# martius-lab/iCEM

Measured on AMD Instinct MI355X. Metric: traj-steps/sec (N x h), iCEM inner planning loop, higher is better.
Workload: dtype f32 storage; model step 2xfp16 planes (3 products), f32 accumulate

## Files before the change

### icem_amd/build.py

```python
import hashlib
import json
import os
import subprocess
import sys
from concurrent.futures import ThreadPoolExecutor

HERE = os.path.dirname(os.path.abspath(__file__))
CSRC = os.path.join(HERE, "csrc")
UNITS = ["generic_kernels.hip", "plan.hip", "abi.hip", "exchange.hip", "k_sample.hip", "k_rollout.hip", "k_merge.hip",
         "k_iter_small.hip", "icem_rssm.hip", "icem_rssm_split.hip", "k_rollout_wide.hip", "collective.hip", "k_rollout_ahead.hip",
         "k_rollout_wide_split.hip", "k_rollout_hn.hip"]
OUT = os.path.join(HERE, "libicem_hip.so")
OUT_FAULTS = os.path.join(HERE, "libicem_hip_faults.so")
FAULT_UNIT = "exchange.hip"
MARK = b"ICEM_BUILD_HASH="
OBJ = os.path.join(CSRC, "_obj")
FLAGS = ["--offload-arch=gfx950", "-O3", "-std=c++17", "-fPIC", "-Wno-unused-function"]
UNIT_FLAGS = {}
if os.environ.get("ICEM_DEV_SHAPES"):
    FLAGS.append(f"-DICEM_FAST_SHAPES(X)=X({os.environ['ICEM_DEV_SHAPES']})")


def _hipcc() -> str:
    return os.environ.get("HIPCC", "/opt/rocm/bin/hipcc")


def _units():
    return [u for u in UNITS if os.path.exists(os.path.join(CSRC, u))]


def _headers():
    hs = sorted(os.path.join(CSRC, f) for f in os.listdir(CSRC) if f.endswith(".h"))
    return hs + [os.path.join(os.path.dirname(HERE), "include", "icem_hip.h")]


def _digest(paths, extra=""):
    m = hashlib.sha256(extra.encode())
    for p in paths:
        m.update(os.path.basename(p).encode())
        with open(p, "rb") as f:
            m.update(f.read())
    return m.hexdigest()[:16]


def source_hash() -> str:
    return _digest([os.path.join(CSRC, u) for u in _units()] + _headers(), " ".join(FLAGS) + repr(sorted(UNIT_FLAGS.items())))


def embedded_hash(path: str = OUT):
    try:
        with open(path, "rb") as f:
            blob = f.read()
    except OSError:
        return None
    at = blob.find(MARK)
    if at < 0:
        return None
    tag = blob[at + len(MARK):at + len(MARK) + 16]
    return tag.decode() if len(tag) == 16 and all(c in b"0123456789abcdef" for c in tag) else None


def build_info() -> dict:
    info = {"source_hash": source_hash(), "built_from": embedded_hash(), "stale": True}
    info["stale"] = info["built_from"] != info["source_hash"]
    return info


def up_to_date() -> bool:
    return not build_info()["stale"]


def _compile(unit, headers_digest, verbose, faults=False):
    src = os.path.join(CSRC, unit)
    extra = [f'-DICEM_BUILD_HASH="{source_hash()}"'] if unit == "abi.hip" else []
    if faults:
        extra.append("-DICEM_FAULT_INJECTION")
    cmd = [_hipcc(), *FLAGS, *UNIT_FLAGS.get(unit, []), *extra, "-I", CSRC, "-c", src]
    key = _digest([src], " ".join(cmd[1:-1]) + headers_digest)
    stem = os.path.splitext(unit)[0] + ("_faults" if faults else "")
    obj = os.path.join(OBJ, f"{stem}.{key}.o")
    if not os.path.exists(obj):
        for f in os.listdir(OBJ):
            if f.startswith(stem + ".") and f.endswith(".o"):
                os.remove(os.path.join(OBJ, f))
        if verbose:
            print(" ".join(cmd + ["-o", obj]), flush=True)
        subprocess.check_call(cmd + ["-o", obj + ".tmp"])
        os.replace(obj + ".tmp", obj)
    return obj


def build(force: bool = False, verbose: bool = True) -> str:
    if not force and up_to_date() and embedded_hash(OUT_FAULTS) == source_hash():
        return OUT
    os.makedirs(OBJ, exist_ok=True)
    if force:
        for f in os.listdir(OBJ):
            os.remove(os.path.join(OBJ, f))
    hd = _digest(_headers())
    with ThreadPoolExecutor(max_workers=min(8, os.cpu_count() or 1)) as ex:
        fut_faults = ex.submit(_compile, FAULT_UNIT, hd, verbose, True)
        objs = list(ex.map(lambda u: _compile(u, hd, verbose), _units()))
        obj_faults = fut_faults.result()
    objs_f = [obj_faults if os.path.basename(o).startswith(os.path.splitext(FAULT_UNIT)[0] + ".") else o for o in objs]
    for out, oo in ((OUT, objs), (OUT_FAULTS, objs_f)):
        cmd = [_hipcc(), "--offload-arch=gfx950", "-shared", "-fPIC", *oo, "-ldl", "-o", out]
        if verbose:
            print(" ".join(cmd), flush=True)
        subprocess.check_call(cmd)
    if embedded_hash() != source_hash():
        raise RuntimeError("libicem_hip.so does not carry the hash of the sources it was just built from")
    return OUT


if __name__ == "__main__":
    build(force="--force" in sys.argv)
    print(json.dumps(build_info()))
```

### icem_amd/csrc/fused_dev.h

```cpp
#pragma once
#include "icem_fused.h"

#include <climits>
#include <cmath>
#include <cstdlib>
#include <algorithm>
#include <type_traits>
#include <utility>

#include "exchange_dev.h"
#include "philox.h"
#include "refit.h"

#ifndef ICEM_FAST_SHAPES
#define ICEM_FAST_SHAPES(X) X(30, 6, 17) X(30, 6, 18) X(12, 6, 17) X(13, 4, 17) X(30, 17, 24)
#endif
#define ICEM_FAST_HORIZONS(X) X(30) X(12) X(13) X(10)

namespace icem {

namespace {

constexpr int HMAX = 32;
constexpr int SWG = 256;
// ... 1036 lines not shown

__device__ __forceinline__ unsigned long long wave_min_u64(unsigned long long x) {
    x = min_dpp<0xB1, 0xF>(x);
    x = min_dpp<0x4E, 0xF>(x);
    x = min_dpp<0x141, 0xF>(x);
    x = min_dpp<0x140, 0xF>(x);
    x = min_dpp<0x142, 0xA>(x);
    x = min_dpp<0x143, 0xC>(x);
    const unsigned lo = __builtin_amdgcn_readlane((int)(unsigned)x, 63);
    const unsigned hi = __builtin_amdgcn_readlane((int)(unsigned)(x >> 32), 63);
    return ((unsigned long long)hi << 32) | lo;
}

template <int CTRL, int ROW_MASK>
__device__ __forceinline__ unsigned min_dpp32(unsigned x) {
    const unsigned o = (unsigned)__builtin_amdgcn_update_dpp((int)x, (int)x, CTRL, ROW_MASK, 0xF, false);
    return o < x ? o : x;
}
__device__ __forceinline__ unsigned wave_min_u32(unsigned x) {
    x = min_dpp32<0xB1, 0xF>(x);
    x = min_dpp32<0x4E, 0xF>(x);
    x = min_dpp32<0x141, 0xF>(x);
    x = min_dpp32<0x140, 0xF>(x);
    x = min_dpp32<0x142, 0xA>(x);
    x = min_dpp32<0x143, 0xC>(x);
    return (unsigned)__builtin_amdgcn_readlane((int)x, 63);
}
__device__ __forceinline__ unsigned long long wave_min_key(unsigned long long x) {
    const unsigned hi = (unsigned)(x >> 32), lo = (unsigned)x;
    const unsigned mh = wave_min_u32(hi);
    const unsigned long long tie = __ballot(hi == mh);
    unsigned ml;
    if (__popcll(tie) == 1)
        ml = (unsigned)__builtin_amdgcn_readlane((int)lo, __ffsll((long long)tie) - 1);
    else
        ml = wave_min_u32(hi == mh ? lo : 0xFFFFFFFFu);
    return ((unsigned long long)mh << 32) | ml;
}

template <int CTRL, int ROW_MASK>
__device__ __forceinline__ unsigned add_dpp(unsigned x) {
    return x + (unsigned)__builtin_amdgcn_update_dpp(0, (int)x, CTRL, ROW_MASK, 0xF, ROW_MASK == 0xF);
}
__device__ __forceinline__ unsigned wave_incl_scan_u32(unsigned x) {
    x = add_dpp<0x111, 0xF>(x);
    x = add_dpp<0x112, 0xF>(x);
    x = add_dpp<0x114, 0xF>(x);
    x = add_dpp<0x118, 0xF>(x);
    x = add_dpp<0x142, 0xA>(x);
    x = add_dpp<0x143, 0xC>(x);
    return x;
}

__device__ __forceinline__ int keep_index0(const MergeSingleArgs& a) { return a.keep_base >= 0 ? a.keep_base : a.n_global; }

template <int KREG>
__device__ __forceinline__ void merge_select(const MergeSingleArgs& a, int lane, unsigned long long* cand,
                                             unsigned long long* sel) {
    unsigned long long k[LPL][KREG];
    const float keep_cost = a.elites_cost_cur ? a.elites_cost_cur[lane < a.n_keep ? lane : 0] : 0.f;
#pragma unroll
    for (int l = 0; l < LPL; ++l) {
        const int list = lane + l * 64;
#pragma unroll
        for (int i = 0; i < KREG; ++i)
            k[l][i] = a.part_k[(size_t)(i < a.K ? i : 0) * a.n_lists + (list < a.n_lists ? list : 0)];
    }
#pragma unroll
    for (int l = 0; l < LPL; ++l) {
        const bool has_list = lane + l * 64 < a.n_lists;
#pragma unroll
        for (int i = 0; i < KREG; ++i) k[l][i] = (has_list && i < a.K) ? k[l][i] : KEY_SENTINEL;
    }
    if (a.dbg && threadIdx.x == 0) a.dbg[1] = wall_clock64();
    if (lane < a.n_keep) {
        unsigned long long v = make_key(keep_cost, keep_index0(a) + lane);
#pragma unroll
        for (int i = 0; i < KREG; ++i) {
            const bool sw = v < k[0][i];
            const unsigned long long t = sw ? k[0][i] : v;
            k[0][i] = sw ? v : k[0][i];
            v = t;
        }
    }
    if (a.dbg && threadIdx.x == 0) a.dbg[2] = wall_clock64();
    unsigned long long mine = k[0][0];
#pragma unroll
    for (int l = 1; l < LPL; ++l) mine = k[l][0] < mine ? k[l][0] : mine;
    const unsigned srt = wave_sort64_u32((unsigned)(mine >> 32), lane);
    const unsigned T = __shfl(srt, a.K - 1, 64);
    unsigned n_cand = 0;
#pragma unroll
    for (int i = 0; i < KREG; ++i) {
        bool p[LPL];
        bool any_lane = false;
#pragma unroll
        for (int l = 0; l < LPL; ++l) {
            p[l] = (unsigned)(k[l][i] >> 32) <= T && k[l][i] != KEY_SENTINEL;
            any_lane |= p[l];
        }
        if (__ballot(any_lane) == 0) break;
#pragma unroll
        for (int l = 0; l < LPL; ++l) {
            const unsigned long long m = __ballot(p[l]);
            if (m != 0) {
                const unsigned pos = n_cand + __builtin_amdgcn_mbcnt_hi((unsigned)(m >> 32), __builtin_amdgcn_mbcnt_lo((unsigned)m, 0u));
                if (p[l] && pos < 64) cand[pos] = k[l][i];
                n_cand += (unsigned)__popcll(m);
            }
        }
    }
    if (a.dbg && threadIdx.x == 0) a.dbg[3] = wall_clock64();
    __builtin_amdgcn_fence(__ATOMIC_SEQ_CST, "workgroup");
    if (n_cand <= 64) {
        unsigned long long key = lane < (int)n_cand ? *((volatile unsigned long long*)&cand[lane]) : KEY_SENTINEL;
        key = wave_sort_n(key, lane, n_cand);
        if (lane < a.K) sel[lane] = key;
    } else {
        for (int r = 0; r < a.K; ++r) {
            unsigned long long head = k[0][0];
#pragma unroll
            for (int l = 1; l < LPL; ++l) head = k[l][0] < head ? k[l][0] : head;
            const unsigned long long best = wave_min_u64(head);
            if (best != KEY_SENTINEL) {
#pragma unroll
                for (int l = 0; l < LPL; ++l) {
                    if (k[l][0] == best) {
#pragma unroll
                        for (int i = 0; i + 1 < KREG; ++i) k[l][i] = k[l][i + 1];
                        k[l][KREG - 1] = KEY_SENTINEL;
                    }
                }
            }
            if (lane == 0) sel[r] = best;
        }
    }
}

__device__ __forceinline__ void merge_select_stream(const MergeSingleArgs& a, int lane, unsigned long long* cand,
                                                    unsigned long long* sel) {
    const int K = a.K, nl = a.n_lists;
    auto key_at = [&](int l, int i) -> unsigned long long {
        const int list = lane + l * 64;
        const unsigned long long v = a.part_k[(size_t)(i < K ? i : 0) * nl + (list < nl ? list : 0)];
        return (list < nl && i < K) ? v : KEY_SENTINEL;
    };
    const unsigned long long kept = lane < a.n_keep ? make_key(a.elites_cost_cur[lane], keep_index0(a) + lane) : KEY_SENTINEL;
    unsigned long long mine = kept;
#pragma unroll
    for (int l = 0; l < LPL; ++l) {
        const unsigned long long v = key_at(l, 0);
        mine = v < mine ? v : mine;
    }
    const unsigned long long srt = wave_sort64(mine, lane);
    const unsigned long long T = __shfl(srt, K - 1, 64);
    unsigned n_cand = 0;
    auto offer = [&](unsigned long long key) {
        const bool p = key <= T && key != KEY_SENTINEL;
        const unsigned long long m = __ballot(p);
        if (m != 0) {
            const unsigned pos = n_cand + __builtin_amdgcn_mbcnt_hi((unsigned)(m >> 32), __builtin_amdgcn_mbcnt_lo((unsigned)m, 0u));
            if (p && pos < 64) cand[pos] = key;
            n_cand += (unsigned)__popcll(m);
        }
        return m != 0;
    };
    offer(kept);
#pragma unroll 1
    for (int l = 0; l < LPL; ++l) {
        if (l * 64 >= nl) break;
#pragma unroll 1
        for (int i = 0; i < K; ++i)
            if (!offer(key_at(l, i))) break;
    }
    __builtin_amdgcn_fence(__ATOMIC_SEQ_CST, "workgroup");
    if (n_cand <= 64) {
        unsigned long long key = lane < (int)n_cand ? *((volatile unsigned long long*)&cand[lane]) : KEY_SENTINEL;
        key = wave_sort_n(key, lane, n_cand);
        if (lane < K) sel[lane] = key;
    } else {
        int cur[LPL];
#pragma unroll
        for (int l = 0; l < LPL; ++l) cur[l] = 0;
        bool kept_live = true;
        for (int r = 0; r < K; ++r) {
            unsigned long long head = kept_live ? kept : KEY_SENTINEL;
#pragma unroll
            for (int l = 0; l < LPL; ++l) {
                const unsigned long long v = key_at(l, cur[l]);
                head = v < head ? v : head;
            }
            const unsigned long long best = wave_min_u64(head);
            if (best != KEY_SENTINEL) {
                if (kept_live && kept == best) kept_live = false;
#pragma unroll
                for (int l = 0; l < LPL; ++l)
                    if (key_at(l, cur[l]) == best) ++cur[l];
            }
            if (lane == 0) sel[r] = best;
        }
    }
}

template <int DEPTH>
__device__ __forceinline__ void merge_select_shallow(const MergeSingleArgs& a, int lane, unsigned long long* cand,
                                                     unsigned long long* sel) {
    const int K = a.K, nl = a.n_lists;
    const float keep_cost = a.elites_cost_cur ? a.elites_cost_cur[lane < a.n_keep ? lane : 0] : 0.f;
    unsigned long long k[LPL][DEPTH];
#pragma unroll
    for (int l = 0; l < LPL; ++l) {
        const int list = lane + l * 64;
#pragma unroll
        for (int i = 0; i < DEPTH; ++i) k[l][i] = a.part_k[(size_t)(i < K ? i : 0) * nl + (list < nl ? list : 0)];
    }
#pragma unroll
    for (int l = 0; l < LPL; ++l) {
        const bool has_list = lane + l * 64 < nl;
#pragma unroll
        for (int i = 0; i < DEPTH; ++i) k[l][i] = (has_list && i < K) ? k[l][i] : KEY_SENTINEL;
    }
    const unsigned long long kept = lane < a.n_keep ? make_key(keep_cost, keep_index0(a) + lane) : KEY_SENTINEL;
    unsigned long long mine = k[0][0];
#pragma unroll
    for (int l = 1; l < LPL; ++l) mine = k[l][0] < mine ? k[l][0] : mine;
    const unsigned srt = wave_sort64_u32((unsigned)(mine >> 32), lane);
    const unsigned T = __shfl(srt, K - 1, 64);
    unsigned n_cand = 0;
    auto offer = [&](unsigned long long key) {
        const bool p = (unsigned)(key >> 32) <= T && key != KEY_SENTINEL;
        const unsigned long long m = __ballot(p);
        if (m != 0) {
            const unsigned pos = n_cand + __builtin_amdgcn_mbcnt_hi((unsigned)(m >> 32), __builtin_amdgcn_mbcnt_lo((unsigned)m, 0u));
            if (p && pos < 64) cand[pos] = key;
            n_cand += (unsigned)__popcll(m);
        }
        return m != 0;
    };
    bool deeper[LPL];
#pragma unroll
    for (int l = 0; l < LPL; ++l) {
        deeper[l] = true;
#pragma unroll
        for (int i = 0; i < DEPTH; ++i)
            if (deeper[l]) deeper[l] = offer(k[l][i]);
    }
#pragma unroll 1
    for (int l = 0; l < LPL; ++l) {
        if (!deeper[l]) continue;
#pragma unroll 1
        for (int i = DEPTH; i < K; ++i) {
            const int list = lane + l * 64;
            const unsigned long long v = list < nl ? a.part_k[(size_t)i * nl + list] : KEY_SENTINEL;
            if (!offer(v)) break;
        }
    }
    offer(kept);
    __builtin_amdgcn_fence(__ATOMIC_SEQ_CST, "workgroup");
    if (n_cand <= 64) {
        unsigned long long key = lane < (int)n_cand ? *((volatile unsigned long long*)&cand[lane]) : KEY_SENTINEL;
        key = wave_sort_n(key, lane, n_cand);
        if (lane < K) sel[lane] = key;
    } else {
        merge_select_stream(a, lane, cand, sel);
    }
}

__device__ __forceinline__ void merge_select_records(const MergeSingleArgs& a, int lane, unsigned long long* cand,
                                                     unsigned long long* sel, int* slot, long long* stamp = nullptr) {
    const int K = a.K, rs = a.h * a.d + 2;
    xchg_wait(a.xw, lane);
    if (stamp && lane == 0) *stamp = wall_clock64();
    auto rec_key = [&](int e) -> unsigned long long {
        if (e >= a.n_rec) return KEY_SENTINEL;
        const float* rec = a.records + (size_t)e * rs;
        return make_key(rec[0], reinterpret_cast<const int*>(rec + 1)[0]);
    };
    unsigned long long k[3] = {rec_key(lane), rec_key(lane + 64),
                               lane < a.n_keep ? make_key(a.elites_cost_cur[lane], a.n_global + lane) : KEY_SENTINEL};
    const unsigned long long k0 = k[0], k1 = k[1], k2 = k[2];
    for (int r = 0; r < K; ++r) {
        unsigned long long head = k[0] < k[1] ? k[0] : k[1];
        head = k[2] < head ? k[2] : head;
        const unsigned long long best = wave_min_key(head);
        if (best != KEY_SENTINEL) {
            if (k0 == best) { slot[r] = lane; k[0] = KEY_SENTINEL; }
            if (k1 == best) { slot[r] = lane + 64; k[1] = KEY_SENTINEL; }
            if (k2 == best) { slot[r] = a.n_rec + lane; k[2] = KEY_SENTINEL; }
        } else if (lane == 0) {
            slot[r] = 0;
        }
        if (lane == 0) sel[r] = best;
    }
    (void)cand;
}

__device__ __forceinline__ void merge_select_records_wg(const MergeSingleArgs& a, bool stager, int lane, int tid, int nthr,
                                                        unsigned long long* sel, int* slot, long long* stamp = nullptr) {
    __shared__ unsigned long long rk_keys[192];
    __shared__ unsigned rk_rank[192];
    const int K = a.K, rs = a.h * a.d + 2;
    if (stager) {
        xchg_wait(a.xw, lane);
        if (stamp && lane == 0) *stamp = wall_clock64();
        auto rec_key = [&](int e) -> unsigned long long {
            if (e >= a.n_rec) return KEY_SENTINEL;
            const float* rec = a.records + (size_t)e * rs;
            return make_key(rec[0], reinterpret_cast<const int*>(rec + 1)[0]);
        };
        rk_keys[lane] = rec_key(lane);
        rk_keys[64 + lane] = rec_key(lane + 64);
        rk_keys[128 + lane] = lane < a.n_keep ? make_key(a.elites_cost_cur[lane], a.n_global + lane) : KEY_SENTINEL;
        rk_rank[lane] = rk_rank[64 + lane] = rk_rank[128 + lane] = 0u;
// ... 9 lines not shown
        const int c = tid % n_live, p = tid / n_live;
        const unsigned long long mine = rk_keys[at(c)];
        unsigned cnt = 0;
        for (int j = p; j < n_live; j += parts) cnt += rk_keys[at(j)] < mine ? 1u : 0u;
        if (cnt) atomicAdd(&rk_rank[at(c)], cnt);
    }
    if (n_live > nthr)
        for (int c = nthr + tid; c < n_live; c += nthr) {
            const unsigned long long mine = rk_keys[at(c)];
            unsigned cnt = 0;
            for (int j = 0; j < n_live; ++j) cnt += rk_keys[at(j)] < mine ? 1u : 0u;
            rk_rank[at(c)] = cnt;
        }
    __syncthreads();
    for (int c = tid; c < n_live; c += nthr) {
        const unsigned long long mine = rk_keys[at(c)];
        const unsigned r = rk_rank[at(c)];
        if (mine != KEY_SENTINEL && r < (unsigned)K) {
            sel[r] = mine;
            slot[r] = c;
        }
    }
    __syncthreads();
}

template <int KREG>
__device__ __forceinline__ void merge_select_split_stage1(const MergeSingleArgs& a, int lane, int w, int nw, unsigned long long* cand ,
                                                          unsigned long long* wsel ) {
    const int per = (a.n_lists + nw - 1) / nw;
    const int base = w * per;
    const int cnt = base < a.n_lists ? (a.n_lists - base < per ? a.n_lists - base : per) : 0;
    const bool has = lane < cnt;
    const int list = has ? base + lane : 0;
    unsigned long long k[KREG];
#pragma unroll
    for (int i = 0; i < KREG; ++i) k[i] = a.part_k[(size_t)(i < a.K ? i : 0) * a.n_lists + list];
#pragma unroll
    for (int i = 0; i < KREG; ++i) k[i] = (has && i < a.K) ? k[i] : KEY_SENTINEL;
    const unsigned srt = wave_sort64_u32((unsigned)(k[0] >> 32), lane);
    const unsigned T = __shfl(srt, a.K - 1, 64);
    unsigned n_cand = 0;
#pragma unroll
    for (int i = 0; i < KREG; ++i) {
        const bool p = (unsigned)(k[i] >> 32) <= T && k[i] != KEY_SENTINEL;
        const unsigned long long m = __ballot(p);
        if (m == 0) break;
        const unsigned pos = n_cand + __builtin_amdgcn_mbcnt_hi((unsigned)(m >> 32), __builtin_amdgcn_mbcnt_lo((unsigned)m, 0u));
        if (p && pos < 64) cand[pos] = k[i];
        n_cand += (unsigned)__popcll(m);
    }
    __builtin_amdgcn_fence(__ATOMIC_SEQ_CST, "workgroup");
    unsigned long long* out = wsel + w * 16;
    if (n_cand <= 64) {
        unsigned long long key = lane < (int)n_cand ? *((volatile unsigned long long*)&cand[lane]) : KEY_SENTINEL;
        key = wave_sort_n(key, lane, n_cand);
        if (lane < 16) out[lane] = lane < a.K ? key : KEY_SENTINEL;
    } else {
        for (int r = 0; r < a.K; ++r) {
            const unsigned long long best = wave_min_u64(k[0]);
            if (best != KEY_SENTINEL && k[0] == best) {
#pragma unroll
                for (int i = 0; i + 1 < KREG; ++i) k[i] = k[i + 1];
                k[KREG - 1] = KEY_SENTINEL;
            }
            if (lane == 0) out[r] = best;
        }
        if (lane >= a.K && lane < 16) out[lane] = KEY_SENTINEL;
    }
}
__device__ __forceinline__ float merge_keep_cost(const MergeSingleArgs& a, int lane) {
    return a.elites_cost_cur ? a.elites_cost_cur[lane < a.n_keep ? lane : 0] : 0.f;
}
__device__ __forceinline__ void merge_select_split_stage2(const MergeSingleArgs& a, int lane, int nw, const unsigned long long* wsel,
                                                          unsigned long long* cand, unsigned long long* sel, float keep_cost) {
    unsigned long long k[5];
#pragma unroll
    for (int j = 0; j < 4; ++j) k[j] = (lane + 64 * j < nw * 16) ? *((volatile const unsigned long long*)&wsel[lane + 64 * j]) : KEY_SENTINEL;
    k[4] = (lane < a.n_keep && a.elites_cost_cur) ? make_key(keep_cost, keep_index0(a) + lane) : KEY_SENTINEL;
    unsigned long long mine = k[0];
#pragma unroll
    for (int j = 1; j < 5; ++j) mine = k[j] < mine ? k[j] : mine;
    const unsigned long long srt = wave_sort64(mine, lane);
    const unsigned long long T = __shfl(srt, a.K - 1, 64);
    unsigned n_cand = 0;
#pragma unroll
    for (int j = 0; j < 5; ++j) {
        const bool p = k[j] <= T && k[j] != KEY_SENTINEL;
        const unsigned long long m = __ballot(p);
        const unsigned pos = n_cand + __builtin_amdgcn_mbcnt_hi((unsigned)(m >> 32), __builtin_amdgcn_mbcnt_lo((unsigned)m, 0u));
        if (p && pos < 64) cand[pos] = k[j];
        n_cand += (unsigned)__popcll(m);
    }
    __builtin_amdgcn_fence(__ATOMIC_SEQ_CST, "workgroup");
    if (n_cand <= 64) {
        unsigned long long key = lane < (int)n_cand ? *((volatile unsigned long long*)&cand[lane]) : KEY_SENTINEL;
        key = wave_sort_n(key, lane, n_cand);
        if (lane < a.K) sel[lane] = key;
    } else {
        for (int r = 0; r < a.K; ++r) {
            unsigned long long head = k[0];
#pragma unroll
            for (int j = 1; j < 5; ++j) head = k[j] < head ? k[j] : head;
            const unsigned long long best = wave_min_u64(head);
            if (best != KEY_SENTINEL) {
#pragma unroll
                for (int j = 0; j < 5; ++j)
                    if (k[j] == best) k[j] = KEY_SENTINEL;
            }
            if (lane == 0) sel[r] = best;
        }
    }
}

template <int NW>
__device__ __forceinline__ bool merge_select_split_by_rank(const MergeSingleArgs& a) { return a.n_keep <= (16 - a.K) * NW; }
template <int NW>
__device__ __forceinline__ float merge_keep_cost_split(const MergeSingleArgs& a, int lane, int w) {
    const int j = w + NW * (lane - a.K);
    return a.elites_cost_cur ? a.elites_cost_cur[(lane >= a.K && lane < 16 && j < a.n_keep) ? j : 0] : 0.f;
}
template <int NW>
__device__ __forceinline__ void merge_select_split_keep(const MergeSingleArgs& a, int lane, int w, unsigned long long* wsel,
                                                        unsigned long long* sel, float keep_cost) {
    if (lane >= a.K && lane < 16) {
        const int j = w + NW * (lane - a.K);
        wsel[w * 16 + lane] = (j < a.n_keep && a.elites_cost_cur) ? make_key(keep_cost, keep_index0(a) + j) : KEY_SENTINEL;
    }
    if (w == 0 && lane < 16) sel[lane] = KEY_SENTINEL;
}
template <int NW>
__device__ __forceinline__ void merge_select_split_rank(const MergeSingleArgs& a, int lane, int w, const unsigned long long* wsel,
                                                        unsigned long long* sel) {
    typedef unsigned long long u64x2 __attribute__((ext_vector_type(2)));
    const int i = lane & 15, q = lane >> 4;
    const unsigned long long mine = wsel[w * 16 + i];
    const u64x2* pairs = reinterpret_cast<const u64x2*>(wsel) + q;
    unsigned place = 0;
#pragma unroll
    for (int c = 0; c < 2 * NW; ++c) {
        const u64x2 b = pairs[4 * c];
        place += (b[0] < mine ? 1u : 0u) + (b[1] < mine ? 1u : 0u);
    }
    place += (unsigned)__shfl_xor((int)place, 16, 64);
    place += (unsigned)__shfl_xor((int)place, 32, 64);
    if (q == 0 && mine != KEY_SENTINEL && place < (unsigned)a.K) sel[place] = mine;
}

template <int KREG, bool REC>
__device__ __forceinline__ void merge_rows(const MergeSingleArgs& a, const unsigned long long* sel, const int* slot,
                                           const float* (&rows)[KREG]) {
    const int hd = a.h * a.d;
    const int lane = (int)(threadIdx.x & 63);
    const int v = REC ? slot[lane < a.K ? lane : 0] : key_idx(sel[lane < a.K ? lane : 0]);
    const float* mine;
    if (REC) mine = v < a.n_rec ? a.records + (size_t)v * (hd + 2) + 2 : a.elites_cur + (size_t)(v - a.n_rec) * hd;
    else mine = v < a.n_pool ? a.actions + (size_t)v * hd : a.elites_cur + (size_t)(v - a.n_global) * hd;
    const unsigned long long bits = (unsigned long long)(size_t)mine;
#pragma unroll
    for (int r = 0; r < KREG; ++r) {
        const int rr = r < a.K ? r : 0;
        const unsigned lo = (unsigned)__builtin_amdgcn_readlane((int)(unsigned)bits, rr);
        const unsigned hi = (unsigned)__builtin_amdgcn_readlane((int)(unsigned)(bits >> 32), rr);
        rows[r] = reinterpret_cast<const float*>((size_t)(((unsigned long long)hi << 32) | lo));
    }
}

template <int H, int D, int ROUNDS, bool RAW>
__device__ __forceinline__ void sample_into_tile(const FastSampleArgs& sa, int n_rows, int r_mine, int jd, float* trow,
                                                 const float* mrow) {
    constexpr int HD = H * D;
    if (r_mine < sa.n) {
        if (RAW) {
            sample_row<H, ROUNDS>(sa.W, (unsigned)(sa.first_index + r_mine), (unsigned)jd, sa.off_lo, sa.off_hi,
                                  sa.seed_lo, sa.seed_hi, [&](int t, float y) { trow[t * D] = y; }, sa.white != 0);
        } else {
            const float lo = sa.low[jd], hi = sa.high[jd];
            sample_row<H, ROUNDS>(sa.W, (unsigned)(sa.first_index + r_mine), (unsigned)jd, sa.off_lo, sa.off_hi,
                                  sa.seed_lo, sa.seed_hi, [&](int t, float y) {
                                      const float v = __builtin_fmaf(y, mrow[HD + t * D], mrow[t * D]);
                                      trow[t * D] = __builtin_amdgcn_fmed3f(v, lo, hi);
                                  }, sa.white != 0);
        }
    } else if (r_mine < n_rows && !RAW) {
        const int e = r_mine - sa.n;
        const float lo = sa.low[jd], hi = sa.high[jd];
        float last = 0.f;
        sample_row<H, ROUNDS>(sa.W, (unsigned)e, (unsigned)jd, sa.off2_lo, sa.off2_hi, sa.seed_lo, sa.seed_hi,
                              [&](int t, float y) {
                                  if (t == H - 1) {
                                      const float v = __builtin_fmaf(y, mrow[HD + t * D], mrow[t * D]);
                                      last = __builtin_amdgcn_fmed3f(v, lo, hi);
                                  }
                              }, sa.white != 0);
        const float* src = sa.elites_src + (size_t)e * HD + jd;
        for (int t = 0; t < H - 1; ++t) trow[t * D] = src[(t + 1) * D];
        trow[(H - 1) * D] = last;
    } else {
        for (int t = 0; t < H; ++t) trow[t * D] = 0.f;
    }
}

template <int H, int D, int ROUNDS, bool RAW, typename Publish>
__device__ __forceinline__ void sample_into_tile_quad(const FastSampleArgs& sa, bool live, int n_rows, int r_mine, int jd, int q,
                                                      float* trow, const float* mrow, const float* Wl, Publish&& publish) {
    constexpr int HD = H * D;
    float g[HMAX];
    const int kind = !live ? 3 : (r_mine < sa.n ? 0 : ((r_mine < n_rows && !RAW) ? 1 : 2));
    if (kind == 0)
        row_normals_quad<H, ROUNDS>((unsigned)(sa.first_index + r_mine), (unsigned)jd, sa.off_lo, sa.off_hi, sa.seed_lo, sa.seed_hi, q, g);
    else if (kind == 1)
        row_normals_quad<H, ROUNDS>((unsigned)(r_mine - sa.n), (unsigned)jd, sa.off2_lo, sa.off2_hi, sa.seed_lo, sa.seed_hi, q, g);
    publish();
    if (kind == 0) {
        if (RAW) {
            row_synth_quad<H>(Wl, g, q, [&](int t, float y) { trow[t * D] = y; }, sa.white != 0);
        } else {
// ... 288 lines not shown
```

### icem_amd/csrc/k_iter_small.hip

```cpp
#include "fused_dev.h"

namespace icem {

namespace {

constexpr bool sr_quad(int d, int rw) { return rw <= 2 && ((4 * 16 * rw * d + 63) / 64) * 64 + 64 <= 1024; }
constexpr int sr_threads(int d, int rw) { return (((sr_quad(d, rw) ? 4 : 1) * 16 * rw * d + 63) / 64) * 64; }

template <int H, int D, int O, int KIND, int ROUNDS, int RW, int KREG, bool REC, int ARITH>
__device__ __forceinline__ void sample_rollout_body(const FastSampleArgs& sa, const FastRolloutArgs& ra, const MergeSingleArgs& am,
                                                    const PackPrev& ap) {
    constexpr bool PM = KREG > 0;
    constexpr bool QS = sr_quad(D, RW);
    constexpr bool T4 = QS && O <= 20 && sr_threads(D, RW) >= 256 * RW && ARITH == 0;
    using T16 = typename TileSel<H, D, O, KIND, ARITH>::type;
    using Tile = typename std::conditional<T4, Tile4<H, D, (O <= 20 ? O : 17), KIND>, T16>::type;
    constexpr int RWV = T4 ? 4 * RW : RW;
    constexpr int HD = H * D;
    constexpr int TPB = 16 * RW;
    constexpr int ROWS = TPB * D;
    constexpr int NT = sr_threads(D, RW);
    constexpr int NTT = NT + (PM ? 64 : 0);
    static_assert(NTT <= 1024 && HD % 2 == 0, "workgroup shape");
    constexpr int VW = HD % 4 == 0 ? 4 : 2;
// ... 13 lines not shown
    const int wave = tid >> 6;
    const int n_rows = ra.n_rows;
    const bool has_pack = PM && REC && ap.part_k != nullptr;
    if constexpr (PM && REC) {
        if (has_pack && blockIdx.x == 0) {
            MergeSingleArgs pk{};
            pk.n_lists = ap.n_lists;
            pk.n_pool = ap.n_pool;
            pk.n_global = ap.n_global;
            pk.K = ap.K;
            pk.h = H;
            pk.d = D;
            pk.part_k = ap.part_k;
            pk.actions = ap.actions;
            pk.n_keep = ap.n_keep;
            pk.elites_cost_cur = ap.keep_costs;
            pk.keep_base = ap.n_loc;
            __builtin_amdgcn_s_setprio(3);
            if (ra.dbg && tid == 0) ra.dbg[0] = wall_clock64();
            if (tid < 64) {
                if constexpr (NTT <= 512)
                    merge_select<12>(pk, lane, cand, sel);
                else
                    merge_select_stream(pk, lane, cand, sel);
            }
            __syncthreads();
            if (ra.dbg && tid == 0) ra.dbg[1] = wall_clock64();
            pack_records_body<12>(pk, ap.n_loc, ap.shard_lo, ap.records, ap.px, tilebuf, sel, tid, NTT);
            if (ra.dbg && tid == 0) ra.dbg[2] = wall_clock64();
            return;
        }
    }
    const int wg = blockIdx.x - (has_pack ? 1 : 0);
    const int n_wg = ra.list_wgs > 0 ? ra.list_wgs : (int)gridDim.x - (has_pack ? 1 : 0);
    const int base = wg * TPB;
    if (base >= n_rows) return;
    if (ra.dbg && tid == 0 && wg == 0) ra.dbg[8] = wall_clock64();
    const int rowi = QS ? tid >> 2 : tid, q = tid & 3;
    const int nl = rowi / D, jd = rowi - nl * D;
    const bool has_row = rowi < ROWS;
    float* trow = tile_rows + nl * HD + jd;
    const float* mrow = ms + jd;
    Tile tile;
    float obs_reg = 0.f;
    constexpr int WPL = (WROWS * HMAX + 63) / 64;
    float wreg[QS ? WPL : 1];
    const bool pre_drawn = !PM && sa.raw_src != nullptr;
    if constexpr (QS) {
        if (tid < NT && !pre_drawn) {
#pragma unroll
            for (int i = 0; i < WPL; ++i) wreg[i] = sa.W[(i * 64 + lane) < WROWS * HMAX ? i * 64 + lane : 0];
        }
    }
    if (!PM) {
        obs_reg = ra.obs0[(tid < 32 && tid < ra.o) ? tid : 0];
        if (wave < RWV) tile.load(ra, lane);
        for (int e = tid; e < HD; e += NTT) {
            ms[e] = sa.mean[e];
            ms[HD + e] = sa.std[e];
        }
        __syncthreads();
    }
    if (ra.dbg && tid == 0 && wg == 0) ra.dbg[9] = wall_clock64();
    const int r_mine = base + nl;
    if (pre_drawn) {
        {
            const int total4 = (n_rows - base < TPB ? n_rows - base : TPB) * (HD / VW);
            const Vec* g4 = reinterpret_cast<const Vec*>(sa.raw_src + (size_t)base * HD);
            Vec* t4 = reinterpret_cast<Vec*>(tile_rows);
            for (int e = tid; e < total4; e += NTT) t4[e] = g4[e];
        }
        __syncthreads();
        if (has_row && tid < NT) {
            const float lo = sa.low[jd], hi = sa.high[jd];
            constexpr int QN = QS ? 4 : 1;
            const int q0 = QS ? q : 0;
            if (r_mine < sa.n) {
                for (int t = q0; t < H; t += QN) {
                    const float v = __builtin_fmaf(trow[t * D], mrow[HD + t * D], mrow[t * D]);
                    trow[t * D] = __builtin_amdgcn_fmed3f(v, lo, hi);
                }
            } else if (r_mine < n_rows) {
                const float* src = sa.elites_src + (size_t)(r_mine - sa.n) * HD + jd;
                if ((H - 1) % QN == q0) {
                    const float v = __builtin_fmaf(trow[(H - 1) * D], mrow[HD + (H - 1) * D], mrow[(H - 1) * D]);
                    trow[(H - 1) * D] = __builtin_amdgcn_fmed3f(v, lo, hi);
                }
                for (int t = q0; t < H - 1; t += QN) trow[t * D] = src[(t + 1) * D];
            } else {
                for (int t = q0; t < H; t += QN) trow[t * D] = 0.f;
            }
        }
    } else
    if constexpr (QS) {
        if (tid < NT) {
            float* wl = Wl[wave];
            sample_into_tile_quad<H, D, ROUNDS, PM>(sa, has_row, n_rows, r_mine, jd, q, trow, mrow, wl, [&]() {
#pragma unroll
                for (int i = 0; i < WPL; ++i) {
                    const int e = i * 64 + lane;
                    if (e < WROWS * HMAX) wl[(e / HMAX) * WQ_STRIDE + (e % HMAX)] = wreg[i];
                }
                __builtin_amdgcn_fence(__ATOMIC_RELEASE, "wavefront");
                __builtin_amdgcn_wave_barrier();
                __builtin_amdgcn_fence(__ATOMIC_ACQUIRE, "wavefront");
            });
        }
    } else if (has_row) {
        sample_into_tile<H, D, ROUNDS, PM>(sa, n_rows, r_mine, jd, trow, mrow);
    }
    if constexpr (PM) {
        if (tid >= NT) {
            if constexpr (RW <= 4) __builtin_amdgcn_s_setprio(3);
            if constexpr (REC) {
                if (ra.dbg && lane == 0 && wg == 0) ra.dbg[3] = wall_clock64();
            }
            else if constexpr (RW >= 8)
                merge_select_stream(am, lane, cand, sel);
            else
                merge_select_shallow<3>(am, lane, cand, sel);
        }
    }
    if (PM) {
        obs_reg = ra.obs0[(tid < 32 && tid < ra.o) ? tid : 0];
        if (wave < RWV) tile.load(ra, lane);
    }
    const float* rd0 = nullptr;
    if constexpr (!T4) rd0 = tile.read_ptr(tilebuf + (wave < RW ? wave : 0) * 16 * HD, lane, HD);
    if constexpr (PM) {
        const MergeSingleArgs& m = am;
        if constexpr (REC) {
            merge_select_records_wg(am, tid >= NT, lane, tid, NTT, sel, slot, (ra.dbg && wg == 0) ? ra.dbg + 7 : nullptr);
            if (ra.dbg && tid == 0 && wg == 0) ra.dbg[4] = wall_clock64();
        } else {
            __syncthreads();
        }
        if (ra.dbg && tid == 0 && wg == 0) ra.dbg[5] = wall_clock64();
        const float* rows[KREG > 0 ? KREG : 1];
        merge_rows<KREG, REC>(m, sel, slot, rows);
        for (int e = tid; e < HD; e += NTT) {
            float xs[KREG > 0 ? KREG : 1];
#pragma unroll
            for (int r = 0; r < KREG; ++r) xs[r] = rows[r][e];
            float nm, ns;
            refit_element_regs<float, KREG>(m.K, m.alpha, m.mean[e], m.std[e], xs, nm, ns);
            ms[e] = nm;
            ms[HD + e] = ns;
            if (wg == 0) {
                m.mean_out[e] = nm;
                m.std_out[e] = ns;
#pragma unroll
                for (int r = 0; r < KREG; ++r)
                    if (r < m.K) m.elites_next[(size_t)r * HD + e] = xs[r];
            }
        }
        if (wg == 0 && tid < m.K) m.elites_cost_next[tid] = key_cost(sel[tid]);
        __syncthreads();
        if (ra.dbg && tid == 0 && wg == 0) ra.dbg[6] = wall_clock64();
        if (has_row && r_mine < sa.n) {
            const float lo = sa.low[jd], hi = sa.high[jd];
            for (int t = QS ? q : 0; t < H; t += QS ? 4 : 1) {
                const float v = __builtin_fmaf(trow[t * D], mrow[HD + t * D], mrow[t * D]);
                trow[t * D] = __builtin_amdgcn_fmed3f(v, lo, hi);
            }
        }
    }
    if (tid < 32) {
        float ov = obs_reg;
        asm volatile("" : "+v"(ov));
        obs_stage[tid] = tid < ra.o ? ov : 0.f;
    }
    if (ra.dbg && tid == 0 && wg == 0) ra.dbg[10] = wall_clock64();
    __syncthreads();
    if (sa.row0_mean && sa.first_index + base == 0) {
        for (int e = tid; e < HD; e += NTT) tile_rows[e] = ms[e];
        __syncthreads();
    }
    {
        const int total4 = (n_rows - base < TPB ? n_rows - base : TPB) * (HD / VW);
        const Vec* t4 = reinterpret_cast<const Vec*>(tile_rows);
        Vec* g4 = reinterpret_cast<Vec*>(sa.out + (size_t)base * HD);
        constexpr int CP0 = (NTT - 64 * RWV >= 128) ? 64 * RWV : 0;
        if (tid >= CP0)
            for (int e = tid - CP0; e < total4; e += NTT - CP0) g4[e] = t4[e];
    }
    if (ra.dbg && tid == 0 && wg == 0) ra.dbg[11] = wall_clock64();
    unsigned long long run_key = KEY_SENTINEL;
    if constexpr (T4) {
        if (wave < RWV) {
            tile.load_obs(obs_stage);
            const int rs = wave * 4 + (lane >> 4);
            const int row = base + rs;
            const float* rd = tile.read_ptr(tilebuf, rs, HD);
            const float* ar = tile.row_ptr(tilebuf, rs, HD);
            typename Tile::State st;
            tile.init(st);
#pragma unroll
            for (int t = 0; t < H; ++t) tile.step(st, rd + t * D, ar + t * D);
            const float cost = tile.cost(st);
            const bool live = row < n_rows;
            if ((lane & 15) == 0) {
                if (live) ra.costs[row] = cost;
                note_nonfinite(ra, cost, live);
                wg_keys[0][0][rs] = (live && row < ra.n_cand) ? make_key(cost, row)
                                    : TPB <= 16 ? KEY_SENTINEL : ((KEY_SENTINEL & 0xFFFFFFFF00000000ull) | (KEY_FILL_LO + (unsigned)rs));
            }
        }
        if (ra.dbg && tid == 0 && wg == 0) ra.dbg[13] = wall_clock64();
        if (ra.K > 0 && wg < n_wg) {
            __syncthreads();
            if (wave == 0 && TPB <= 16) {
                const unsigned long long key = wave_sort_first<16>(lane < TPB ? wg_keys[0][0][lane] : KEY_SENTINEL, lane);
                if (lane < ra.K) {
// ... 224 lines not shown
```

### icem_amd/csrc/k_merge.hip

```cpp
#include "fused_dev.h"
#include "refit.h"

namespace icem {

namespace {

template <int KREG, bool REC>
__device__ __forceinline__ void merge_single_body(const MergeSingleArgs& a, unsigned char* smem_raw) {
    __shared__ unsigned long long sel[64];
    __shared__ unsigned long long cand[64];
    __shared__ int slot[64];
    float* new_mean = reinterpret_cast<float*>(smem_raw);
    const int tid = threadIdx.x;
    const int lane = tid & 63;
    const int hd = a.h * a.d;
    if (a.dbg && threadIdx.x == 0) a.dbg[0] = wall_clock64();
    constexpr int EPL = 4;
    const bool pre = hd <= MERGE_WG * EPL;
    float om[EPL], os[EPL];
#pragma unroll
    for (int i = 0; i < EPL; ++i) {
        const int e = tid + i * MERGE_WG;
        om[i] = (pre && e < hd) ? a.mean[e] : 0.f;
        os[i] = (pre && e < hd) ? a.std[e] : 0.f;
    }
    if constexpr (REC) {
        merge_select_records_wg(a, tid < 64, lane, tid, MERGE_WG, sel, slot);
        if (a.dbg && threadIdx.x == 0) a.dbg[4] = wall_clock64();
    } else {
        if (tid < 64) merge_select_shallow<3>(a, lane, cand, sel);
        if (a.dbg && threadIdx.x == 0) a.dbg[4] = wall_clock64();
        __syncthreads();
    }
    const float* rows[KREG];
    merge_rows<KREG, REC>(a, sel, slot, rows);
    auto finish_one = [&](int e, float old_mean, float old_std) {
        float xs[KREG];
#pragma unroll
        for (int r = 0; r < KREG; ++r) xs[r] = rows[r][e];
#pragma unroll
        for (int r = 0; r < KREG; ++r)
            if (r < a.K) a.elites_next[(size_t)r * hd + e] = xs[r];
        float nm, ns;
        refit_element_regs<float, KREG>(a.K, a.alpha, old_mean, old_std, xs, nm, ns);
        if (!a.last) {
            a.mean_out[e] = nm;
            a.std_out[e] = ns;
        } else {
            new_mean[e] = nm;
        }
    };
    if (pre) {
#pragma unroll
        for (int i = 0; i < EPL; ++i) {
            const int e = tid + i * MERGE_WG;
            if (e < hd) finish_one(e, om[i], os[i]);
        }
    } else {
        for (int e = tid; e < hd; e += MERGE_WG) finish_one(e, a.mean[e], a.std[e]);
    }
    if (a.dbg && threadIdx.x == 0) a.dbg[5] = wall_clock64();
    if (tid < a.K) a.elites_cost_next[tid] = key_cost(sel[tid]);
    if (a.last) {
        __syncthreads();
        for (int e = tid; e < hd; e += MERGE_WG) {
            const int j = e % a.d;
            a.mean_out[e] = (e + a.d < hd) ? new_mean[e + a.d] : new_mean[e];
            a.std_out[e] = (a.high[j] - a.low[j]) / 2.f * a.init_std;
        }
        if (tid < a.d) a.executed[tid] = rows[0][tid];
        if (tid == 0) a.best_cost[0] = key_cost(sel[0]);
    }
    if (a.dbg && threadIdx.x == 0) a.dbg[6] = wall_clock64();
}

template <int KREG, bool REC>
__global__ __launch_bounds__(MERGE_WG) void merge_single_kernel(MergeSingleArgs a) {
    extern __shared__ __attribute__((aligned(16))) unsigned char smem_raw[];
    merge_single_body<KREG, REC>(a, smem_raw);
}

template <int H, int KREG>
__global__ __launch_bounds__(MERGE_WG) void merge_noise_kernel(MergeSingleArgs a, FastSampleArgs z1, FastSampleArgs z2, int wgs1) {
    extern __shared__ __attribute__((aligned(16))) unsigned char smem_raw[];
    if (blockIdx.x == 0) {
        merge_single_body<KREG, false>(a, smem_raw);
        return;
    }
    const bool second = (int)blockIdx.x > wgs1;
    const FastSampleArgs& z = second ? z2 : z1;
    float* tile = reinterpret_cast<float*>(smem_raw);
    const int d = z.d, hd = H * d, tpw = MERGE_WG / d, tid = threadIdx.x;
    const int n_base = ((int)blockIdx.x - 1 - (second ? wgs1 : 0)) * tpw;
    const int n_here = cmin(tpw, z.n - n_base);
    if (tid < n_here * d) {
        const int nl = tid / d;
        const int j = tid - nl * d;
        float* trow = tile + nl * hd + j;
        sample_row<H, 10>(z.W, (unsigned)(z.first_index + n_base + nl), (unsigned)j, z.off_lo, z.off_hi, z.seed_lo, z.seed_hi,
                          [&](int t, float y) { trow[t * d] = y; }, z.white != 0);
    }
    __syncthreads();
    float* gdst = z.out + (size_t)n_base * hd;
    const int total = n_here * hd;
    if ((hd & 3) == 0) {
        const float4* t4 = reinterpret_cast<const float4*>(tile);
        float4* g4 = reinterpret_cast<float4*>(gdst);
        for (int e = tid; e < total / 4; e += MERGE_WG) g4[e] = t4[e];
    } else {
        for (int e = tid; e < total; e += MERGE_WG) gdst[e] = tile[e];
    }
}

template <int H, int KREG>
__global__ __launch_bounds__(MERGE_WG) void merge_noise_batch_kernel(const MergeNoiseBatchArgs* __restrict__ args, BatchBases bases, int wgs1) {
    extern __shared__ __attribute__((aligned(16))) unsigned char smem_raw[];
    const MergeNoiseBatchArgs& g = args[blockIdx.y];
    if (blockIdx.x == 0) {
        const MergeSingleArgs a = from_device(g.a);
        merge_single_body<KREG, false>(a, smem_raw);
        return;
    }
    const bool second = (int)blockIdx.x > wgs1;
// ... 222 lines not shown
```

Before: 7.397 billion.

## Prefetch merge and sample inputs into registers ahead of syncs and selection

In the small-iteration kernel, mean/std, low/high bounds, raw noise rows and shifted elite values are now loaded into registers before the barrier, so the pre-drawn tile copy no longer needs its own barrier and global loads overlap. In the merge kernel, bounds are requested while the selection wave works, the executed action comes from a register instead of re-reading row 0, and the new-mean scratch and reread helpers use explicit LDS/global address spaces. A branchless keep-cost load and an extra object-path helper in the build script are also added. The cost is higher register pressure, which could lower occupancy.

```diff
diff --git a/icem_amd/build.py b/icem_amd/build.py
--- a/icem_amd/build.py
+++ b/icem_amd/build.py
@@ -70,7 +70,7 @@
     return not build_info()["stale"]
 
 
-def _compile(unit, headers_digest, verbose, faults=False):
+def _object(unit, headers_digest, faults=False):
     src = os.path.join(CSRC, unit)
     extra = [f'-DICEM_BUILD_HASH="{source_hash()}"'] if unit == "abi.hip" else []
     if faults:
@@ -78,7 +78,16 @@
     cmd = [_hipcc(), *FLAGS, *UNIT_FLAGS.get(unit, []), *extra, "-I", CSRC, "-c", src]
     key = _digest([src], " ".join(cmd[1:-1]) + headers_digest)
     stem = os.path.splitext(unit)[0] + ("_faults" if faults else "")
-    obj = os.path.join(OBJ, f"{stem}.{key}.o")
+    return cmd, os.path.join(OBJ, f"{stem}.{key}.o")
+
+
+def object_path(unit: str) -> str:
+    return _object(unit, _digest(_headers()))[1]
+
+
+def _compile(unit, headers_digest, verbose, faults=False):
+    cmd, obj = _object(unit, headers_digest, faults)
+    stem = os.path.splitext(unit)[0] + ("_faults" if faults else "")
     if not os.path.exists(obj):
         for f in os.listdir(OBJ):
             if f.startswith(stem + ".") and f.endswith(".o"):
diff --git a/icem_amd/csrc/fused_dev.h b/icem_amd/csrc/fused_dev.h
--- a/icem_amd/csrc/fused_dev.h
+++ b/icem_amd/csrc/fused_dev.h
@@ -1112,13 +1112,27 @@
     return x;
 }
 
+__device__ __forceinline__ unsigned long long lds_reread_u64(const unsigned long long* p) {
+#ifdef ICEM_DEBUG
+    if (!__builtin_amdgcn_is_shared(p)) __builtin_trap();
+#endif
+    return *(const volatile __attribute__((address_space(3))) unsigned long long*)p;
+}
+
 __device__ __forceinline__ int keep_index0(const MergeSingleArgs& a) { return a.keep_base >= 0 ? a.keep_base : a.n_global; }
+
+__device__ __forceinline__ float merge_keep_cost(const MergeSingleArgs& a, int lane) {
+    const bool has = a.elites_cost_cur != nullptr;
+    const float* src = has ? a.elites_cost_cur : reinterpret_cast<const float*>(a.part_k);
+    const float v = src[(has && lane < a.n_keep) ? lane : 0];
+    return has ? v : 0.f;
+}
 
 template <int KREG>
 __device__ __forceinline__ void merge_select(const MergeSingleArgs& a, int lane, unsigned long long* cand,
                                              unsigned long long* sel) {
     unsigned long long k[LPL][KREG];
-    const float keep_cost = a.elites_cost_cur ? a.elites_cost_cur[lane < a.n_keep ? lane : 0] : 0.f;
+    const float keep_cost = merge_keep_cost(a, lane);
 #pragma unroll
     for (int l = 0; l < LPL; ++l) {
         const int list = lane + l * 64;
@@ -1173,7 +1187,7 @@
     if (a.dbg && threadIdx.x == 0) a.dbg[3] = wall_clock64();
     __builtin_amdgcn_fence(__ATOMIC_SEQ_CST, "workgroup");
     if (n_cand <= 64) {
-        unsigned long long key = lane < (int)n_cand ? *((volatile unsigned long long*)&cand[lane]) : KEY_SENTINEL;
+        unsigned long long key = lane < (int)n_cand ? lds_reread_u64(&cand[lane]) : KEY_SENTINEL;
         key = wave_sort_n(key, lane, n_cand);
         if (lane < a.K) sel[lane] = key;
     } else {
@@ -1235,7 +1249,7 @@
     }
     __builtin_amdgcn_fence(__ATOMIC_SEQ_CST, "workgroup");
     if (n_cand <= 64) {
-        unsigned long long key = lane < (int)n_cand ? *((volatile unsigned long long*)&cand[lane]) : KEY_SENTINEL;
+        unsigned long long key = lane < (int)n_cand ? lds_reread_u64(&cand[lane]) : KEY_SENTINEL;
         key = wave_sort_n(key, lane, n_cand);
         if (lane < K) sel[lane] = key;
     } else {
@@ -1266,7 +1280,7 @@
 __device__ __forceinline__ void merge_select_shallow(const MergeSingleArgs& a, int lane, unsigned long long* cand,
                                                      unsigned long long* sel) {
     const int K = a.K, nl = a.n_lists;
-    const float keep_cost = a.elites_cost_cur ? a.elites_cost_cur[lane < a.n_keep ? lane : 0] : 0.f;
+    const float keep_cost = merge_keep_cost(a, lane);
     unsigned long long k[LPL][DEPTH];
 #pragma unroll
     for (int l = 0; l < LPL; ++l) {
@@ -1318,7 +1332,7 @@
     offer(kept);
     __builtin_amdgcn_fence(__ATOMIC_SEQ_CST, "workgroup");
     if (n_cand <= 64) {
-        unsigned long long key = lane < (int)n_cand ? *((volatile unsigned long long*)&cand[lane]) : KEY_SENTINEL;
+        unsigned long long key = lane < (int)n_cand ? lds_reread_u64(&cand[lane]) : KEY_SENTINEL;
         key = wave_sort_n(key, lane, n_cand);
         if (lane < K) sel[lane] = key;
     } else {
@@ -1434,7 +1448,7 @@
     __builtin_amdgcn_fence(__ATOMIC_SEQ_CST, "workgroup");
     unsigned long long* out = wsel + w * 16;
     if (n_cand <= 64) {
-        unsigned long long key = lane < (int)n_cand ? *((volatile unsigned long long*)&cand[lane]) : KEY_SENTINEL;
+        unsigned long long key = lane < (int)n_cand ? lds_reread_u64(&cand[lane]) : KEY_SENTINEL;
         key = wave_sort_n(key, lane, n_cand);
         if (lane < 16) out[lane] = lane < a.K ? key : KEY_SENTINEL;
     } else {
@@ -1450,14 +1464,11 @@
         if (lane >= a.K && lane < 16) out[lane] = KEY_SENTINEL;
     }
 }
-__device__ __forceinline__ float merge_keep_cost(const MergeSingleArgs& a, int lane) {
-    return a.elites_cost_cur ? a.elites_cost_cur[lane < a.n_keep ? lane : 0] : 0.f;
-}
 __device__ __forceinline__ void merge_select_split_stage2(const MergeSingleArgs& a, int lane, int nw, const unsigned long long* wsel,
                                                           unsigned long long* cand, unsigned long long* sel, float keep_cost) {
     unsigned long long k[5];
 #pragma unroll
-    for (int j = 0; j < 4; ++j) k[j] = (lane + 64 * j < nw * 16) ? *((volatile const unsigned long long*)&wsel[lane + 64 * j]) : KEY_SENTINEL;
+    for (int j = 0; j < 4; ++j) k[j] = (lane + 64 * j < nw * 16) ? lds_reread_u64(&wsel[lane + 64 * j]) : KEY_SENTINEL;
     k[4] = (lane < a.n_keep && a.elites_cost_cur) ? make_key(keep_cost, keep_index0(a) + lane) : KEY_SENTINEL;
     unsigned long long mine = k[0];
 #pragma unroll
@@ -1475,7 +1486,7 @@
     }
     __builtin_amdgcn_fence(__ATOMIC_SEQ_CST, "workgroup");
     if (n_cand <= 64) {
-        unsigned long long key = lane < (int)n_cand ? *((volatile unsigned long long*)&cand[lane]) : KEY_SENTINEL;
+        unsigned long long key = lane < (int)n_cand ? lds_reread_u64(&cand[lane]) : KEY_SENTINEL;
         key = wave_sort_n(key, lane, n_cand);
         if (lane < a.K) sel[lane] = key;
     } else {
@@ -1537,13 +1548,14 @@
     const float* mine;
     if (REC) mine = v < a.n_rec ? a.records + (size_t)v * (hd + 2) + 2 : a.elites_cur + (size_t)(v - a.n_rec) * hd;
     else mine = v < a.n_pool ? a.actions + (size_t)v * hd : a.elites_cur + (size_t)(v - a.n_global) * hd;
+    typedef const float __attribute__((address_space(1))) * GRow;
     const unsigned long long bits = (unsigned long long)(size_t)mine;
 #pragma unroll
     for (int r = 0; r < KREG; ++r) {
         const int rr = r < a.K ? r : 0;
         const unsigned lo = (unsigned)__builtin_amdgcn_readlane((int)(unsigned)bits, rr);
         const unsigned hi = (unsigned)__builtin_amdgcn_readlane((int)(unsigned)(bits >> 32), rr);
-        rows[r] = reinterpret_cast<const float*>((size_t)(((unsigned long long)hi << 32) | lo));
+        rows[r] = (const float*)reinterpret_cast<GRow>((size_t)(((unsigned long long)hi << 32) | lo));
     }
 }
 
diff --git a/icem_amd/csrc/k_iter_small.hip b/icem_amd/csrc/k_iter_small.hip
--- a/icem_amd/csrc/k_iter_small.hip
+++ b/icem_amd/csrc/k_iter_small.hip
@@ -89,27 +89,76 @@
             for (int i = 0; i < WPL; ++i) wreg[i] = sa.W[(i * 64 + lane) < WROWS * HMAX ? i * 64 + lane : 0];
         }
     }
+    const int r_mine = base + nl;
+    float lo_reg = 0.f, hi_reg = 0.f;
+    if ((PM || pre_drawn) && tid < NT) {
+        lo_reg = sa.low[jd];
+        hi_reg = sa.high[jd];
+    }
+    constexpr int NVR = !PM ? (TPB * (HD / VW) + NTT - 1) / NTT : 1;
+    constexpr int NVB = NVR < 4 ? NVR : 4;
+    constexpr int NEL = !PM && QS ? (H - 1 + 3) / 4 : 1;
+    typedef float RawV __attribute__((ext_vector_type(VW)));
+    RawV rawv[NVB];
+    float elv[NEL];
     if (!PM) {
+        const int total4 = (n_rows - base < TPB ? n_rows - base : TPB) * (HD / VW);
+        RawV* t4 = reinterpret_cast<RawV*>(tile_rows);
+        float mreg[(HD + NTT - 1) / NTT], sreg[(HD + NTT - 1) / NTT];
+#pragma unroll
+        for (int i = 0; i < (HD + NTT - 1) / NTT; ++i) {
+            const int e = tid + i * NTT;
+            mreg[i] = sa.mean[e < HD ? e : 0];
+            sreg[i] = sa.std[e < HD ? e : 0];
+        }
+        if (pre_drawn) {
+            const RawV* g4 = reinterpret_cast<const RawV*>(sa.raw_src + (size_t)base * HD);
+#pragma unroll
+            for (int i = 0; i < NVB; ++i) {
+                const int e = tid + i * NTT;
+                rawv[i] = g4[e < total4 ? e : 0];
+            }
+            if constexpr (QS) {
+                if (has_row && tid < NT && r_mine >= sa.n && r_mine < n_rows) {
+                    const float* src = sa.elites_src + (size_t)(r_mine - sa.n) * HD + jd;
+#pragma unroll
+                    for (int i = 0; i < NEL; ++i) elv[i] = src[(q + 4 * i < H - 1 ? q + 4 * i + 1 : 1) * D];
+                }
+            }
+        }
         obs_reg = ra.obs0[(tid < 32 && tid < ra.o) ? tid : 0];
         if (wave < RWV) tile.load(ra, lane);
-        for (int e = tid; e < HD; e += NTT) {
-            ms[e] = sa.mean[e];
-            ms[HD + e] = sa.std[e];
+#pragma unroll
+        for (int i = 0; i < (HD + NTT - 1) / NTT; ++i) {
+            const int e = tid + i * NTT;
+            if (e < HD) {
+                ms[e] = mreg[i];
+                ms[HD + e] = sreg[i];
+            }
+        }
+        if (pre_drawn) {
+#pragma unroll
+            for (int i = 0; i < NVB; ++i) {
+                const int e = tid + i * NTT;
+                if (e < total4) t4[e] = rawv[i];
+            }
+            if constexpr (NVR > NVB) {
+                const RawV* g4 = reinterpret_cast<const RawV*>(sa.raw_src + (size_t)base * HD);
+                for (int e0 = tid + NVB * NTT; e0 < total4; e0 += NVB * NTT) {
+#pragma unroll
+                    for (int i = 0; i < NVB; ++i) rawv[i] = g4[e0 + i * NTT < total4 ? e0 + i * NTT : 0];
+#pragma unroll
+                    for (int i = 0; i < NVB; ++i)
+                        if (e0 + i * NTT < total4) t4[e0 + i * NTT] = rawv[i];
+                }
+            }
         }
         __syncthreads();
     }
     if (ra.dbg && tid == 0 && wg == 0) ra.dbg[9] = wall_clock64();
-    const int r_mine = base + nl;
     if (pre_drawn) {
-        {
-            const int total4 = (n_rows - base < TPB ? n_rows - base : TPB) * (HD / VW);
-            const Vec* g4 = reinterpret_cast<const Vec*>(sa.raw_src + (size_t)base * HD);
-            Vec* t4 = reinterpret_cast<Vec*>(tile_rows);
-            for (int e = tid; e < total4; e += NTT) t4[e] = g4[e];
-        }
-        __syncthreads();
         if (has_row && tid < NT) {
-            const float lo = sa.low[jd], hi = sa.high[jd];
+            const float lo = lo_reg, hi = hi_reg;
             constexpr int QN = QS ? 4 : 1;
             const int q0 = QS ? q : 0;
             if (r_mine < sa.n) {
@@ -123,7 +172,13 @@
                     const float v = __builtin_fmaf(trow[(H - 1) * D], mrow[HD + (H - 1) * D], mrow[(H - 1) * D]);
                     trow[(H - 1) * D] = __builtin_amdgcn_fmed3f(v, lo, hi);
                 }
-                for (int t = q0; t < H - 1; t += QN) trow[t * D] = src[(t + 1) * D];
+                if constexpr (QS) {
+#pragma unroll
+                    for (int i = 0; i < NEL; ++i)
+                        if (q + 4 * i < H - 1) trow[(q + 4 * i) * D] = elv[i];
+                } else {
+                    for (int t = q0; t < H - 1; t += QN) trow[t * D] = src[(t + 1) * D];
+                }
             } else {
                 for (int t = q0; t < H; t += QN) trow[t * D] = 0.f;
             }
@@ -173,6 +228,7 @@
             __syncthreads();
         }
         if (ra.dbg && tid == 0 && wg == 0) ra.dbg[5] = wall_clock64();
+        if (!REC && ra.dbg && tid == 0 && wg == 0) ra.dbg[15] = wall_clock64();
         const float* rows[KREG > 0 ? KREG : 1];
         merge_rows<KREG, REC>(m, sel, slot, rows);
         for (int e = tid; e < HD; e += NTT) {
@@ -194,8 +250,9 @@
         if (wg == 0 && tid < m.K) m.elites_cost_next[tid] = key_cost(sel[tid]);
         __syncthreads();
         if (ra.dbg && tid == 0 && wg == 0) ra.dbg[6] = wall_clock64();
+        if (!REC && ra.dbg && tid == 0 && wg == 0) ra.dbg[7] = wall_clock64();
         if (has_row && r_mine < sa.n) {
-            const float lo = sa.low[jd], hi = sa.high[jd];
+            const float lo = lo_reg, hi = hi_reg;
             for (int t = QS ? q : 0; t < H; t += QS ? 4 : 1) {
                 const float v = __builtin_fmaf(trow[t * D], mrow[HD + t * D], mrow[t * D]);
                 trow[t * D] = __builtin_amdgcn_fmed3f(v, lo, hi);
diff --git a/icem_amd/csrc/k_merge.hip b/icem_amd/csrc/k_merge.hip
--- a/icem_amd/csrc/k_merge.hip
+++ b/icem_amd/csrc/k_merge.hip
@@ -10,45 +10,60 @@
     __shared__ unsigned long long sel[64];
     __shared__ unsigned long long cand[64];
     __shared__ int slot[64];
-    float* new_mean = reinterpret_cast<float*>(smem_raw);
+    typedef float __attribute__((address_space(3))) * LdsF;
+    const LdsF new_mean = (LdsF)smem_raw;
     const int tid = threadIdx.x;
     const int lane = tid & 63;
     const int hd = a.h * a.d;
     if (a.dbg && threadIdx.x == 0) a.dbg[0] = wall_clock64();
     constexpr int EPL = 4;
     const bool pre = hd <= MERGE_WG * EPL;
-    float om[EPL], os[EPL];
+    float om[EPL], os[EPL], blo[EPL], bhi[EPL];
 #pragma unroll
     for (int i = 0; i < EPL; ++i) {
         const int e = tid + i * MERGE_WG;
         om[i] = (pre && e < hd) ? a.mean[e] : 0.f;
         os[i] = (pre && e < hd) ? a.std[e] : 0.f;
     }
+    auto request_bounds = [&]() {
+#pragma unroll
+        for (int i = 0; i < EPL; ++i) {
+            const int e = tid + i * MERGE_WG;
+            blo[i] = (pre && a.last && e < hd) ? a.low[e % a.d] : 0.f;
+            bhi[i] = (pre && a.last && e < hd) ? a.high[e % a.d] : 0.f;
+        }
+    };
+    if (REC || tid >= 64) request_bounds();
     if constexpr (REC) {
         merge_select_records_wg(a, tid < 64, lane, tid, MERGE_WG, sel, slot);
         if (a.dbg && threadIdx.x == 0) a.dbg[4] = wall_clock64();
     } else {
         if (tid < 64) merge_select_shallow<3>(a, lane, cand, sel);
         if (a.dbg && threadIdx.x == 0) a.dbg[4] = wall_clock64();
+        if (tid < 64) request_bounds();
         __syncthreads();
     }
     const float* rows[KREG];
     merge_rows<KREG, REC>(a, sel, slot, rows);
+    float best0 = 0.f;
     auto finish_one = [&](int e, float old_mean, float old_std) {
         float xs[KREG];
 #pragma unroll
         for (int r = 0; r < KREG; ++r) xs[r] = rows[r][e];
 #pragma unroll
+        for (int r = 0; r < KREG; ++r) asm volatile("" : "+v"(xs[r]));
+        float nm, ns;
+        refit_element_regs<float, KREG>(a.K, a.alpha, old_mean, old_std, xs, nm, ns);
+#pragma unroll
         for (int r = 0; r < KREG; ++r)
             if (r < a.K) a.elites_next[(size_t)r * hd + e] = xs[r];
-        float nm, ns;
-        refit_element_regs<float, KREG>(a.K, a.alpha, old_mean, old_std, xs, nm, ns);
         if (!a.last) {
             a.mean_out[e] = nm;
             a.std_out[e] = ns;
         } else {
             new_mean[e] = nm;
         }
+        if (e == tid) best0 = xs[0];
     };
     if (pre) {
 #pragma unroll
@@ -63,12 +78,23 @@
     if (tid < a.K) a.elites_cost_next[tid] = key_cost(sel[tid]);
     if (a.last) {
         __syncthreads();
-        for (int e = tid; e < hd; e += MERGE_WG) {
-            const int j = e % a.d;
-            a.mean_out[e] = (e + a.d < hd) ? new_mean[e + a.d] : new_mean[e];
-            a.std_out[e] = (a.high[j] - a.low[j]) / 2.f * a.init_std;
-        }
-        if (tid < a.d) a.executed[tid] = rows[0][tid];
+        if (pre) {
+#pragma unroll
+            for (int i = 0; i < EPL; ++i) {
+                const int e = tid + i * MERGE_WG;
+                if (e < hd) {
+                    a.mean_out[e] = (e + a.d < hd) ? new_mean[e + a.d] : new_mean[e];
+                    a.std_out[e] = (bhi[i] - blo[i]) / 2.f * a.init_std;
+                }
+            }
+        } else {
+            for (int e = tid; e < hd; e += MERGE_WG) {
+                const int j = e % a.d;
+                a.mean_out[e] = (e + a.d < hd) ? new_mean[e + a.d] : new_mean[e];
+                a.std_out[e] = (a.high[j] - a.low[j]) / 2.f * a.init_std;
+            }
+        }
+        if (tid < a.d) a.executed[tid] = best0;
         if (tid == 0) a.best_cost[0] = key_cost(sel[0]);
     }
     if (a.dbg && threadIdx.x == 0) a.dbg[6] = wall_clock64();
```

Measured after the change: 7.637 billion, median of 6. +3.2%, better.
